# JitongZ/shockwave-replication

Hardware: AMD Instinct MI355X
Metric: Shockwave plan solves/sec at 900 jobs x 30 rounds (higher is better)
Workload: dtype f64 objective / fp32 ranking keys

## Files before the change

### shockwave-replication_amd/csrc/sw_block.h

```cpp
#pragma once
#include <hip/hip_runtime.h>
#include <stdint.h>

#define SW_BLOCK 512
#define SW_WAVES (SW_BLOCK / 64)

template <int NW>
struct sw_xchg_t {
    int64_t i[2][NW][2];
    double d[2][NW][2];
    uint64_t u[2][NW];
    uint64_t u2[2][NW][2];
    int32_t s[2][NW];
};
using sw_xchg = sw_xchg_t<SW_WAVES>;

__device__ __forceinline__ int lane_id() { return threadIdx.x & 63; }
__device__ __forceinline__ int wave_id() { return threadIdx.x >> 6; }

__device__ __forceinline__ int32_t sw_u32(int32_t x) { return __builtin_amdgcn_readfirstlane(x); }
__device__ __forceinline__ uint64_t sw_u64(uint64_t x) {
    const uint32_t lo = (uint32_t)__builtin_amdgcn_readfirstlane((int)(uint32_t)x);
    const uint32_t hi = (uint32_t)__builtin_amdgcn_readfirstlane((int)(uint32_t)(x >> 32));
    return ((uint64_t)hi << 32) | lo;
}
__device__ __forceinline__ int64_t sw_i64(int64_t x) { return (int64_t)sw_u64((uint64_t)x); }
__device__ __forceinline__ double sw_f64u(double x) {
    return __builtin_bit_cast(double, sw_u64(__builtin_bit_cast(uint64_t, x)));
}

__device__ __forceinline__ void wave_sync() {
    __builtin_amdgcn_fence(__ATOMIC_SEQ_CST, "wavefront");
    __builtin_amdgcn_wave_barrier();
}

__device__ __forceinline__ int32_t dpp_incscan_i32(int32_t x) {
    x += __builtin_amdgcn_update_dpp(0, x, 0x111, 0xF, 0xF, false);
    x += __builtin_amdgcn_update_dpp(0, x, 0x112, 0xF, 0xF, false);
    x += __builtin_amdgcn_update_dpp(0, x, 0x114, 0xF, 0xF, false);
    x += __builtin_amdgcn_update_dpp(0, x, 0x118, 0xF, 0xF, false);
    x += __builtin_amdgcn_update_dpp(0, x, 0x142, 0xA, 0xF, false);
    x += __builtin_amdgcn_update_dpp(0, x, 0x143, 0xC, 0xF, false);
    return x;
}
__device__ __forceinline__ int32_t dpp_incmax_i32(int32_t x) {
    const int32_t lo = INT32_MIN;
    int32_t y;
    y = __builtin_amdgcn_update_dpp(lo, x, 0x111, 0xF, 0xF, false); x = y > x ? y : x;
    y = __builtin_amdgcn_update_dpp(lo, x, 0x112, 0xF, 0xF, false); x = y > x ? y : x;
    y = __builtin_amdgcn_update_dpp(lo, x, 0x114, 0xF, 0xF, false); x = y > x ? y : x;
    y = __builtin_amdgcn_update_dpp(lo, x, 0x118, 0xF, 0xF, false); x = y > x ? y : x;
    y = __builtin_amdgcn_update_dpp(lo, x, 0x142, 0xA, 0xF, false); x = y > x ? y : x;
    y = __builtin_amdgcn_update_dpp(lo, x, 0x143, 0xC, 0xF, false); x = y > x ? y : x;
    return x;
}
__device__ __forceinline__ int32_t wave_sum_i32(int32_t v) {
    return __builtin_amdgcn_readlane(dpp_incscan_i32(v), 63);
}
__device__ __forceinline__ int32_t wave_max_i32(int32_t v) {
    return __builtin_amdgcn_readlane(dpp_incmax_i32(v), 63);
}
__device__ __forceinline__ int32_t wave_min_i32(int32_t v) {
    return -wave_max_i32(-v);
}
__device__ __forceinline__ int32_t wave_incscan_i32(int32_t v) { return dpp_incscan_i32(v); }
__device__ __forceinline__ int32_t wave_sufscan_i32(int32_t v) {
    const int32_t inc = dpp_incscan_i32(v);
    return __builtin_amdgcn_readlane(inc, 63) - inc + v;
}

#define SW_DPP64(x, idv, ctrl, rm)                                                              \
    ((((uint64_t)(uint32_t)__builtin_amdgcn_update_dpp((int)(uint32_t)((idv) >> 32),            \
                                                       (int)(uint32_t)((x) >> 32), ctrl, rm,    \
                                                       0xF, false)) << 32) |                    \
     (uint64_t)(uint32_t)__builtin_amdgcn_update_dpp((int)(uint32_t)(idv), (int)(uint32_t)(x),  \
                                                     ctrl, rm, 0xF, false))
#define SW_DPP64_STEPS(STEP) STEP(0x111, 0xF) STEP(0x112, 0xF) STEP(0x114, 0xF) STEP(0x118, 0xF) \
    STEP(0x142, 0xA) STEP(0x143, 0xC)

__device__ __forceinline__ uint64_t sw_readlane63_u64(uint64_t x) {
    const uint32_t lo = (uint32_t)__builtin_amdgcn_readlane((int)(uint32_t)x, 63);
    const uint32_t hi = (uint32_t)__builtin_amdgcn_readlane((int)(uint32_t)(x >> 32), 63);
    return ((uint64_t)hi << 32) | lo;
}
__device__ __forceinline__ uint64_t wave_max_u64(uint64_t x) {
#define SW_MAXU_(c, rm)                               \
    {                                                 \
        const uint64_t y_ = SW_DPP64(x, 0ull, c, rm); \
        x = y_ > x ? y_ : x;                          \
    }
    SW_DPP64_STEPS(SW_MAXU_)
#undef SW_MAXU_
    return sw_readlane63_u64(x);
}
__device__ __forceinline__ uint64_t wave_min_u64(uint64_t x) {
#define SW_MINU_(c, rm)                                \
    {                                                  \
        const uint64_t y_ = SW_DPP64(x, ~0ull, c, rm); \
        x = y_ < x ? y_ : x;                           \
    }
    SW_DPP64_STEPS(SW_MINU_)
#undef SW_MINU_
    return sw_readlane63_u64(x);
}
__device__ __forceinline__ double wave_max_f64(double v) {
    uint64_t x = __builtin_bit_cast(uint64_t, v);
#define SW_MAXD_(c, rm)                                                       \
    {                                                                         \
        const uint64_t y_ = SW_DPP64(x, 0xFFF0000000000000ull, c, rm);        \
        x = __builtin_bit_cast(double, y_) > __builtin_bit_cast(double, x) ? y_ : x; \
    }
    SW_DPP64_STEPS(SW_MAXD_)
#undef SW_MAXD_
    return __builtin_bit_cast(double, sw_readlane63_u64(x));
}

__device__ __forceinline__ double wave_min_f64(double v) {
    uint64_t x = __builtin_bit_cast(uint64_t, v);
#define SW_MIND_(c, rm)                                                       \
    {                                                                         \
        const uint64_t y_ = SW_DPP64(x, 0x7FF0000000000000ull, c, rm);        \
        x = __builtin_bit_cast(double, y_) < __builtin_bit_cast(double, x) ? y_ : x; \
    }
    SW_DPP64_STEPS(SW_MIND_)
#undef SW_MIND_
    return __builtin_bit_cast(double, sw_readlane63_u64(x));
}

template <typename T>
__device__ __forceinline__ T wave_sum(T v) {
#pragma unroll
    for (int o = 32; o >= 1; o >>= 1) v += __shfl_xor(v, o, 64);
    return v;
}

template <typename T>
__device__ __forceinline__ T wave_max(T v) {
#pragma unroll
    for (int o = 32; o >= 1; o >>= 1) {
        T x = __shfl_xor(v, o, 64);
        v = x > v ? x : v;
    }
    return v;
}

template <typename T>
__device__ __forceinline__ T wave_min(T v) {
#pragma unroll
    for (int o = 32; o >= 1; o >>= 1) {
        T x = __shfl_xor(v, o, 64);
        v = x < v ? x : v;
    }
    return v;
}

template <typename T>
__device__ __forceinline__ T wave_incscan(T v) {
    const int lane = lane_id();
#pragma unroll
    for (int o = 1; o < 64; o <<= 1) {
        T y = __shfl_up(v, o, 64);
        if (lane >= o) v += y;
    }
    return v;
}

template <typename T>
__device__ __forceinline__ T wave_sufscan(T v) {
    const int lane = lane_id();
#pragma unroll
    for (int o = 1; o < 64; o <<= 1) {
        T y = __shfl_down(v, o, 64);
        if (lane + o < 64) v += y;
    }
    return v;
}

__device__ __forceinline__ int32_t wave_sort_asc_i32(int32_t v) {
    const int lane = lane_id();
#pragma unroll
    for (int k = 2; k <= 64; k <<= 1) {
#pragma unroll
        for (int j = k >> 1; j > 0; j >>= 1) {
            const int32_t o = __shfl_xor(v, j, 64);
            const bool up = (lane & k) == 0;
// ... 274 lines not shown
```

### shockwave-replication_amd/csrc/sw_kernels.hip

```cpp
#include <hip/hip_runtime.h>
#include <stdint.h>

#include "../../include/shockwave_amd.h"
#include "sw_arith.h"
#include "sw_rowsearch.h"
#include "sw_block.h"
#include "sw_device.h"
#include "sw_pack.h"
#include "sw_bnb.h"
#include "sw_repair.h"
#include "sw_reround_dev.h"
#include "sw_p2x_inst.h"

namespace {

#ifdef SW_STAMPS
#define SW_STAMP(slot)                                                            \
    do {                                                                          \
        __syncthreads();                                                          \
        if (threadIdx.x == 0 && B.stamps) {                                       \
            uint64_t now_ = __builtin_amdgcn_s_memtime();                         \
            B.stamps[(size_t)inst_ * SW_STAMP_SLOTS + (slot)] += now_ - stamp_prev_;      \
            stamp_prev_ = now_;                                                   \
        }                                                                         \
// ... 1706 lines not shown
        v.bound = bound;
        v.passes = c.passes;
        B.lvl[inst_] = v;
    }
}

__device__ __forceinline__ void emit_plan_bytes(uint8_t* plan, const uint64_t* ym, int N, int T) {
    const int32_t nbytes = N * T;
    const int32_t mis = (int32_t)(reinterpret_cast<uintptr_t>(plan) & 15u);
    const int32_t head = min(nbytes, (16 - mis) & 15);
    const int32_t nch = (nbytes - head) >> 4;
    auto byte_at = [&](int32_t b) {
        const int32_t j = b / T;
        return (uint8_t)((ym[j] >> (b - j * T)) & 1ull);
    };
    for (int32_t b = threadIdx.x; b < head; b += SW_BLOCK) plan[b] = byte_at(b);
    for (int32_t b = head + nch * 16 + threadIdx.x; b < nbytes; b += SW_BLOCK) plan[b] = byte_at(b);
    uint4* dst = reinterpret_cast<uint4*>(plan + head);
    for (int32_t ci = threadIdx.x; ci < nch; ci += SW_BLOCK) {
        const int32_t b0 = head + ci * 16;
        int32_t j = b0 / T, t = b0 - j * T;
        uint64_t m = ym[j];
        uint32_t wv[4] = {0u, 0u, 0u, 0u};
#pragma unroll
        for (int k = 0; k < 16; ++k) {
            wv[k >> 2] |= (uint32_t)((m >> t) & 1ull) << ((k & 3) * 8);
            if (++t == T) {
                t = 0;
                ++j;
                if (k < 15 && j < N) m = ym[j];
            }
        }
        dst[ci] = make_uint4(wv[0], wv[1], wv[2], wv[3]);
    }
}

__device__ __forceinline__ void emit_out(sw_out_dev* out, double U, double M, double k, double P2,
                                         double bound, int64_t passes, int32_t status) {
    sw_out_dev o;
    o.objective = U - k * M;
    o.utility = U;
    o.makespan = M;
    o.p2_objective = P2;
    o.bound = bound;
    o.iters = (int32_t)passes;
    o.status = status | (sw_p1_uncertified(o.objective, bound) ? SW_STATUS_P1_UNCERTIFIED : 0);
    *out = o;
}

static_assert(SW_LDS_JOBS <= (1 << 11), "the job index fits the position word");
#define SW_LWA_MARKED (-1)

template <bool WS>
__device__ __forceinline__ const uint64_t* pack_instance(const sw_batch_dev& B, unsigned char* smem, int inst_) {
    const sw_inst_dev* I = &B.inst[inst_];
    Ctx<32, true, true> c;
    c.init(B, I);
    const sw_lvl_dev lv = B.lvl[inst_];
    c.passes = lv.passes;
    const int64_t jo = I->job_off;
    constexpr sw_pack_carve O = sw_pack_offsets();
    c.blk.X = (sw_xchg*)(smem + O.X);
    c.set_pack_lds(smem + O.PL);
    c.misc = (int64_t*)(smem + O.misc);
    c.rep = (sw_repair_t*)(smem + O.rep);
    c.nbest = smem + O.nbest;
    c.placed = smem + O.placed;
    c.placed2 = smem + O.placed2;
    c.ycur = (uint64_t*)(smem + O.ycur);
    c.y2 = (uint64_t*)(smem + O.y2);
    c.sbuf = (uint64_t*)(smem + O.sbuf);
    sw_out_dev* out = &B.out[inst_];
    if constexpr (!WS) {
        int64_t act_l = 0;
        c.for_jobs([&](int j, int s) {
            (void)s;
            c.nbest[j] = B.nb[jo + j];
            act_l += c.nbest[j] > 0;
        });
        if (c.blk.sum(act_l) > SW_BLOCK) {
            if (threadIdx.x == 0) out->status = SW_STATUS_SLOW_MARK;
            return nullptr;
        }
        c.pack(4, c.nbest, c.ycur, c.placed);
    } else {
        const int A_ = sw_u32(B.lwa[inst_]);
        if (A_ == SW_LWA_MARKED) return nullptr;
        c.for_jobs([&](int j, int s) {
            (void)s;
            c.nbest[j] = B.nb[jo + j];
            c.ycur[j] = 0;
        });
        const bool mine = (int)threadIdx.x < A_;
        const uint32_t word = mine ? B.lws[jo + threadIdx.x] : 0u;
        const uint64_t mk1 = mine ? B.lwm[jo + threadIdx.x] : 0ull;
        c.pack_back(4, c.nbest, c.ycur, c.placed, mine, (int)(word >> 16), word & 0xFFFFu, mk1);
    }
    int64_t def_l = 0;
    c.for_jobs([&](int j, int s) {
        (void)s;
        def_l += (int64_t)c.w_in[j] * (c.nbest[j] - c.placed[j]);
    });
    int64_t dfc = c.blk.sum(def_l);
    c.passes++;
    int32_t status = 0;
    if (dfc != 0 && c.repair_pack(c.nbest, c.ycur, c.placed, c.y2, c.placed2)) {
        c.for_jobs([&](int j, int s) {
            (void)s;
            c.ycur[j] = c.y2[j];
        });
        c.passes++;
        dfc = 0;
        status |= SW_STATUS_P2_REPAIRED;
    }
    if (dfc != 0) {
        if (threadIdx.x == 0) out->status = SW_STATUS_SLOW_MARK;
        return nullptr;
    }
    int64_t any_l = 0;
    double p2 = 0.0;
    c.for_jobs([&](int j, int s) {
        (void)s;
        const uint64_t m = c.ycur[j];
        const int cnt = __popcll(m);
        any_l += (cnt > 0);
        p2 = p2 + (cnt > 0 ? sw_p2_term(m, cnt, c.p_in[j]) : 0.0);
        B.planned[jo + j] = cnt;
    });
    const double P2 = c.blk.detsum(p2);
    const int64_t any_n = c.blk.sum(any_l);
    if (any_n == 0) status |= SW_STATUS_NO_PLANNED;
    if (threadIdx.x == 0) emit_out(out, lv.U, lv.M, c.k, P2, lv.bound, c.passes, status);
    return c.ycur;
}

__device__ __forceinline__ void pack_tail(const sw_batch_dev& B, const uint64_t* ym, unsigned char* smem,
                                          int inst) {
    const sw_inst_dev* I = &B.inst[inst];
    sw_out_dev* out = &B.out[inst];
    const int N = I->N, T = I->T, G = I->G;
    const int64_t jo = I->job_off;
    const int q = (N + SW_BLOCK - 1) / SW_BLOCK;
    const int j0 = sw_tid_opaque() * q, j1 = min(j0 + q, N);
    __syncthreads();
    int act = 0;
#pragma unroll
    for (int k = 0; k < 2; ++k) act += (j0 + k < j1 && ym[j0 + k] != 0ull) ? 1 : 0;
    const bool run = B.fuse_p2x && !(out->status & SW_STATUS_P2_FALLBACK);
    sw_p2x_lds* L = reinterpret_cast<sw_p2x_lds*>(smem);
    const size_t Lsz = SW_P2X_VAR_OFF;
    unsigned char* var = smem + Lsz;
    static_assert(offsetof(sw_p2x_lds, X) + sizeof(sw_xchg) <= sw_pack_offsets().ycur,
                  "the pack's masks lie past the exchange words of sw_p2x_lds");
    sw_blk blk;
    blk.X = &L->X;
    blk.par = 0;
    int A = 0;
    const int a0 = blk.exscan(act, A);
    A = __builtin_amdgcn_readfirstlane(A);
    const uint64_t* yemit = ym;
    if (run && A > 0 && A <= SW_P2X_AMAX) {
        const size_t vb = (sw_p2x_var_bytes(A, T) + 15) & ~(size_t)15;
        const bool onchip = Lsz + vb + (size_t)SW_P2X_ARR_BYTES * A <= (size_t)B.lds_bytes &&
                            var + vb >= reinterpret_cast<const unsigned char*>(ym + N);
        unsigned char* base = onchip ? var + vb : B.p2ws + (size_t)SW_P2X_ARR_BYTES * jo;
        const size_t n = onchip ? (size_t)A : (size_t)N;
        const sw_p2x_arrays X = sw_p2x_view(base, n);
        for (int k = 0, a = a0; k < 2; ++k) {
            if (j0 + k >= j1) break;
            const uint64_t m = ym[j0 + k];
            if (m == 0ull) continue;
            const int j = j0 + k;
            X.cw[a] = B.w[jo + j];
            X.cj[a] = j;
            X.cc[a] = B.p[jo + j] / (double)__popcll(m);
            X.cm[a] = m;
            ++a;
        }
        __syncthreads();
#ifdef SW_STAMPS
        uint64_t* sp = B.stamps ? B.stamps + (size_t)inst * SW_STAMP_SLOTS + 32 : nullptr;
#else
        uint64_t* sp = nullptr;
#endif
        const int nc = sw_p2x_block<SW_WAVES>(blk, L, var, X, A, T, G, sp);
        __syncthreads();
        int act2 = 0;
        for (int j = j0r(N); j < j1r(N); ++j) act2 += B.planned[jo + j] > 0;
        int A2;
        int a = blk.exscan(act2, A2);
        uint64_t mf[2];
        double acc = 0.0;
#pragma unroll
        for (int k = 0; k < 2; ++k) {
            const int j = j0r(N) + k;
            mf[k] = 0ull;
            if (j >= j1r(N)) continue;
            if (B.planned[jo + j] <= 0) {
                acc = acc + 0.0;
                continue;
            }
            mf[k] = X.cm[a++];
            acc = acc + sw_p2_term(mf[k], __popcll(mf[k]), B.p[jo + j]);
        }
        if (nc > 0) {
            const double P2 = blk.detsum(acc);
            if (threadIdx.x == 0) {
                out->p2_objective = P2;
                out->status |= SW_STATUS_P2_EXCHANGED;
            }
        }
        __syncthreads();
        uint64_t* yf = reinterpret_cast<uint64_t*>(smem);
#pragma unroll
        for (int k = 0; k < 2; ++k)
            if (j0r(N) + k < j1r(N)) yf[j0r(N) + k] = mf[k];
        yemit = yf;
        __syncthreads();
    }
    if (B.want_masks)
        for (int j = j0r(N); j < j1r(N); ++j) B.masks[jo + j] = yemit[j];
    emit_plan_bytes(B.plan + I->plan_off, yemit, N, T);
}

template <int KT, bool ONE>
struct RREnv {
    Ctx<KT, ONE>& c;
    sw_blk& blk;
    int N, T, G;
    double k;
    uint8_t *S, *Sb;
    uint32_t* items;
    double *iv, *dpA, *dpB;
    uint64_t* bits;
    double rv[SW_JPT], r0[SW_JPT], r1[SW_JPT];
    double *gv, *g0, *g1;
    __device__ RREnv(Ctx<KT, ONE>& cc) : c(cc), blk(cc.blk) {}
    template <class F>
    __device__ __forceinline__ void for_jobs(F&& f) { c.for_jobs(f); }
    __device__ __forceinline__ sw_jobc jc(int j) const { return c.jc(j, 0); }
    __device__ __forceinline__ double f(const sw_jobc& q, int n) const {
        return sw_f(&q, n, c.nb, c.beta, c.ell, c.slope);
    }
    __device__ __forceinline__ bool tj(int j) const { return c.jc(j, 0).w <= G; }
    __device__ __forceinline__ uint64_t& y(int j) { return c.ybest[j]; }
    __device__ __forceinline__ int cnt(int j) const { return c.nfin[j]; }
    __device__ __forceinline__ void add_cnt(int j, int d) { c.nfin[j] = (uint8_t)(c.nfin[j] + d); }
    __device__ __forceinline__ double& V(int j, int s) {
        if constexpr (ONE) { (void)j; return rv[s]; } else { (void)s; return gv[j]; }
    }
    __device__ __forceinline__ double& H0(int j, int s) {
        if constexpr (ONE) { (void)j; return r0[s]; } else { (void)s; return g0[j]; }
    }
    __device__ __forceinline__ double& H1(int j, int s) {
        if constexpr (ONE) { (void)j; return r1[s]; } else { (void)s; return g1[j]; }
    }
};

template <int KT, bool ONE>
__device__ __forceinline__ int reround(Ctx<KT, ONE>& c, double* rr_dpA, double* rr_dpB, uint64_t* rr_bits) {
    RREnv<KT, ONE> e(c);
    e.N = c.N;
    e.T = c.T;
    e.G = c.G;
    e.k = c.k;
    e.S = c.placed;
    e.Sb = c.placed2;
    if constexpr (ONE) {
// ... 386 lines not shown
```

### shockwave-replication_amd/csrc/sw_p2x_dev.h

```cpp
#pragma once
#include <hip/hip_runtime.h>
#include <stdint.h>

#include "../../include/shockwave_amd.h"
#include "sw_arith.h"
#include "sw_block.h"
#include "sw_device.h"
#include "sw_p2x.h"

struct sw_p2x_arrays {
    int32_t* cw;
    int32_t* cj;
    double* cc;
    uint64_t* cm;
};
static_assert(SW_P2X_ARR_BYTES == 2 * sizeof(int32_t) + sizeof(double) + sizeof(uint64_t),
              "SW_P2X_ARR_BYTES (sw_p2x.h) must cover the sw_p2x_arrays layout");

struct sw_p2x_pre {
    const int32_t* hdr;
    const int32_t* ord;
    const double* pc;
    const uint64_t* B;
    const double* Wb;
    const int8_t* Wk;
};
enum { SW_P2X_HDR_K = 0, SW_P2X_HDR_WC = 1, SW_P2X_HDR_M = 9, SW_P2X_HDR_OFF = 17,
       SW_P2X_HDR_NW = 26, SW_P2X_HDR_BOFF = 34, SW_P2X_HDR_A = 42, SW_P2X_HDR_INTS = 48 };

struct sw_p2x_lds {
    sw_xchg X;
    int32_t wc[SW_P2X_KMAX], M[SW_P2X_KMAX], off[SW_P2X_KMAX + 1], nw[SW_P2X_KMAX],
        boff[SW_P2X_KMAX];
    int32_t K, len, nrec, pad;
    uint64_t touched;
    uint32_t wmap[8];
    int32_t room[SW_TMAX];
    int32_t pr[SW_TMAX + 1];
    int32_t cyc[SW_TMAX + 2];
    double delta;
    double bd[SW_TMAX + 1];
    int32_t bp[SW_TMAX + 1];
    double pv[SW_WAVES][64];
    int8_t pt[SW_WAVES][64];
    int32_t bfdone;
    int32_t fq[SW_P2X_KMAX];
    double dw[SW_P2X_KMAX][SW_TMAX + 1];
};

__host__ __device__ inline size_t sw_p2x_var_bytes(int maxA, int T) {
    const size_t a = (size_t)(maxA < SW_P2X_AMAX ? maxA : SW_P2X_AMAX);
    const size_t words = (size_t)T * ((a + 63) / 64 + SW_P2X_KMAX);
    size_t np = 1;
    while (np < a) np <<= 1;
    const size_t work = words * 8 + (size_t)T * T * 8 + (((size_t)T * T + 15) & ~(size_t)15) +
                        (size_t)SW_P2X_MAX_MOVES * 4;
    return a * 8 + ((a * 4 + 15) & ~(size_t)15) + (work > 16 * np ? work : 16 * np);
}

static __device__ __forceinline__ int p2x_class(const sw_p2x_lds* L, int32_t w) {
    int k = 0;
    while (k < L->K - 1 && L->wc[k] != w) ++k;
    return k;
}

static __device__ __forceinline__ void p2x_find_cycle(sw_p2x_lds* L, const double* W, int T, int F,
                                                      double* dw, bool warm, uint64_t (&acc)[11]) {
    const int tid = threadIdx.x, lane = lane_id(), wv = wave_id();
    (void)acc;
#ifdef SW_STAMPS
    uint64_t bt_ = __builtin_amdgcn_s_memtime();
#define BF_STAMP(k)                                                   \
    do {                                                              \
        const uint64_t now_ = __builtin_amdgcn_s_memtime();           \
        acc[k] += now_ - bt_;                                         \
        bt_ = now_;                                                   \
    } while (0)
#else
#define BF_STAMP(k) \
    do {            \
    } while (0)
#endif
    const bool act = lane < T;
    if (tid <= T) {
        L->bd[tid] = warm ? dw[tid] : 0.0;
        L->bp[tid] = -1;
    }
    if (tid == 0) L->bfdone = 0;
    const bool roomok = wv == 0 && act && L->room[lane] >= F;
    const bool anyroom = __ballot(roomok) != 0;
    const int nq = (T + SW_WAVES - 1) / SW_WAVES;
    int ndbl = 0;
    while ((1 << ndbl) < T + 1) ++ndbl;
    __syncthreads();
    for (int it = 0; it <= T; ++it) {
#ifdef SW_STAMPS
        acc[7] += 1;
#endif
        BF_STAMP(10);
        {
            const int ul = act ? lane : 0;
            const int t0 = wv * nq, t1 = min(T, t0 + nq);
            double cb = SW_P2X_NONE;
            int ct = 0;
            for (int t = t0; t < t1; ++t) {
                const double w = W[t * T + ul];
                const double v = L->bd[t] + w;
                const bool take = w < SW_P2X_NONE && v < cb;
                cb = take ? v : cb;
                ct = take ? t : ct;
            }
            L->pv[wv][lane] = cb;
            L->pt[wv][lane] = (int8_t)ct;
        }
        __syncthreads();
        BF_STAMP(9);
        if (wv == 0) {
            __builtin_amdgcn_s_setprio(3);
            double d = act ? L->bd[lane] : 0.0;
// ... 223 lines not shown
        sp_t_ = now_;                                                \
    } while (0)
#else
#define P2X_STAMP(k) \
    do {             \
    } while (0)
#endif

template <int NT, int EMAX>
static __device__ __forceinline__ void p2x_sort_regs(uint64_t (&hi)[EMAX], uint64_t (&lo)[EMAX], int E,
                                                     int np, uint64_t* xs) {
    const int tid = threadIdx.x;
    for (int kk = 2; kk <= np; kk <<= 1) {
        for (int jj = kk >> 1; jj > 0; jj >>= 1) {
            if (jj < E) {
#pragma unroll
                for (int e = 0; e < EMAX; ++e) {
                    const int f = e ^ jj;
                    if (e < E && f > e) {
                        const int i = tid * E + e;
                        const bool up = (i & kk) == 0;
                        uint64_t ah = hi[e], al = lo[e], bh = 0, bl = 0;
#pragma unroll
                        for (int g = 0; g < EMAX; ++g)
                            if (g == f) { bh = hi[g]; bl = lo[g]; }
                        const bool gt = ah > bh || (ah == bh && al > bl);
                        if (up == gt) {
                            hi[e] = bh; lo[e] = bl;
#pragma unroll
                            for (int g = 0; g < EMAX; ++g)
                                if (g == f) { hi[g] = ah; lo[g] = al; }
                        }
                    }
                }
            } else {
                uint64_t ph[EMAX], pl[EMAX];
                const int dj = jj / E;
                if (dj < 64) {
#pragma unroll
                    for (int e = 0; e < EMAX; ++e) {
                        ph[e] = __shfl_xor(hi[e], dj, 64);
                        pl[e] = __shfl_xor(lo[e], dj, 64);
                    }
                } else {
                    if (tid * E < np)
                        for (int e = 0; e < E; ++e) {
                            xs[tid * E + e] = hi[e];
                            xs[np + tid * E + e] = lo[e];
                        }
                    __syncthreads();
                    const int pt = tid ^ dj;
                    if (tid * E < np)
                        for (int e = 0; e < E; ++e) {
                            ph[e] = xs[pt * E + e];
                            pl[e] = xs[np + pt * E + e];
                        }
                    __syncthreads();
                }
                const bool lower = (tid & dj) == 0;
#pragma unroll
                for (int e = 0; e < EMAX; ++e) {
                    if (e >= E) continue;
                    const int i = tid * E + e;
                    const bool up = (i & kk) == 0;
                    const bool gt = hi[e] > ph[e] || (hi[e] == ph[e] && lo[e] > pl[e]);
                    if ((lower == up) ? gt : !gt) {
                        hi[e] = ph[e];
                        lo[e] = pl[e];
                    }
                }
            }
        }
    }
}

struct sw_p2x_state {
    int K;
    double* pc;
    int32_t* ord;
    uint64_t* B;
    double* W;
    int8_t* Wk;
    double delta;
};

static __device__ __forceinline__ void p2x_load_size(sw_p2x_lds* L, int K, int F) {
    const int tid = threadIdx.x;
    if (tid < SW_P2X_KMAX) {
        const int wk = tid < K ? L->wc[tid] : 0;
        L->fq[tid] = (wk > 0 && wk <= F && F % wk == 0 && F / wk <= SW_P2X_QMAX) ? F / wk : 0;
    }
}

template <int NW, int EMAX = 1, bool SETUP_ONLY = false>
__device__ __forceinline__ int sw_p2x_block(sw_blk_t<NW>& blk, sw_p2x_lds* L, unsigned char* var,
                                            const sw_p2x_arrays& X, int A, int T, int G,
                                            uint64_t* sp = nullptr, const sw_p2x_pre* pre = nullptr,
                                            sw_p2x_state* st = nullptr) {
    constexpr int NT = NW * 64;
    const int tid = threadIdx.x;
    (void)sp;
    uint64_t sp_a_[11] = {0, 0, 0, 0, 0, 0, 0, 0, 0, 0, 0};
#ifdef SW_STAMPS
    uint64_t sp_t_ = __builtin_amdgcn_s_memtime();
#endif
    if (A <= 0 || T < 2 || A > SW_P2X_AMAX) return 0;
    if (pre && pre->hdr[SW_P2X_HDR_K] < 0) return 0;
    if (pre) {
        if (tid < SW_P2X_KMAX) {
            L->wc[tid] = pre->hdr[SW_P2X_HDR_WC + tid];
            L->M[tid] = pre->hdr[SW_P2X_HDR_M + tid];
            L->nw[tid] = pre->hdr[SW_P2X_HDR_NW + tid];
            L->boff[tid] = pre->hdr[SW_P2X_HDR_BOFF + tid];
        }
        if (tid <= SW_P2X_KMAX) L->off[tid] = pre->hdr[SW_P2X_HDR_OFF + tid];
        if (tid == 0) L->K = pre->hdr[SW_P2X_HDR_K];
        __syncthreads();
    }
    if (!pre) {
    if (tid < 8) L->wmap[tid] = 0u;
    __syncthreads();
    for (int a = tid; a < A; a += NT) atomicOr(&L->wmap[X.cw[a] >> 5], 1u << (X.cw[a] & 31));
    __syncthreads();
    if (tid == 0) {
        int K = 0;
        for (int i = 0; i < 8; ++i) K += __builtin_popcount(L->wmap[i]);
        if (K > SW_P2X_KMAX) {
            L->K = -1;
        } else {
            K = 0;
            for (int i = 0; i < 8; ++i)
                for (uint32_t b = L->wmap[i]; b; b &= b - 1) L->wc[K++] = 32 * i + __builtin_ctz(b);
            L->K = K;
            for (int k = 0; k < K; ++k) L->M[k] = 0;
        }
    }
    __syncthreads();
    if (L->K < 0) return 0;
    for (int a = tid; a < A; a += NT) atomicAdd(&L->M[p2x_class(L, X.cw[a])], 1);
    __syncthreads();
    if (tid == 0) {
        const int K = L->K;
        int o = 0, b = 0;
        for (int k = 0; k < K; ++k) {
            L->off[k] = o;
            L->nw[k] = (L->M[k] + 63) / 64;
            L->boff[k] = b;
            o += L->M[k];
            b += L->nw[k] * T;
        }
        L->off[K] = o;
    }
    }
    const int K = L->K;
    P2X_STAMP(0);
    double* pc = reinterpret_cast<double*>(var);
    int32_t* ord = reinterpret_cast<int32_t*>(var + (size_t)A * 8);
    unsigned char* vb = var + (size_t)A * 8 + (((size_t)A * 4 + 15) & ~(size_t)15);
    __syncthreads();
    const int nwords = L->boff[K - 1] + L->nw[K - 1] * T;
    uint64_t* B = reinterpret_cast<uint64_t*>(vb);
    double* W = reinterpret_cast<double*>(vb + (size_t)nwords * 8);
    int8_t* Wk = reinterpret_cast<int8_t*>(W + T * T);
    int32_t* rec = reinterpret_cast<int32_t*>(reinterpret_cast<unsigned char*>(Wk) + ((T * T + 15) & ~15));
    if (pre) {
        for (int p = tid; p < A; p += NT) {
            ord[p] = pre->ord[p];
            pc[p] = pre->pc[p];
        }
        for (int i = tid; i < nwords; i += NT) B[i] = pre->B[i];
        __syncthreads();
    } else if (A <= NT) {
        int np = 1;
        while (np < A) np <<= 1;
        uint64_t hi = ~0ull, lo = ~0ull;
        if (tid < A) {
            const uint64_t ck = sw_p2x_ckey(X.cc[tid]);
            hi = ((uint64_t)p2x_class(L, X.cw[tid]) << 61) | (~ck & ((1ull << 61) - 1));
            lo = ((uint64_t)(uint32_t)X.cj[tid] << 32) | (uint32_t)tid;
        }
        uint64_t* xs = reinterpret_cast<uint64_t*>(vb);
        for (int kk = 2; kk <= np; kk <<= 1) {
            for (int jj = kk >> 1; jj > 0; jj >>= 1) {
                uint64_t ph = ~0ull, pl = ~0ull;
                if (jj >= 64) {
                    if (tid < np) {
                        xs[tid] = hi;
                        xs[np + tid] = lo;
                    }
                    __syncthreads();
                    if (tid < np) {
                        ph = xs[tid ^ jj];
                        pl = xs[np + (tid ^ jj)];
                    }
                    __syncthreads();
                } else {
                    ph = __shfl_xor(hi, jj, 64);
                    pl = __shfl_xor(lo, jj, 64);
                }
                const bool up = (tid & kk) == 0, lower = (tid & jj) == 0;
                const bool gt = hi > ph || (hi == ph && lo > pl);
                if ((lower == up) ? gt : !gt) {
                    hi = ph;
                    lo = pl;
                }
            }
        }
        if (tid < A) {
            const int a = (int)(uint32_t)lo;
            ord[tid] = a;
            pc[tid] = X.cc[a];
        }
        __syncthreads();
    } else if (EMAX > 1 && A <= EMAX * NT) {
        int np = 1;
        while (np < A) np <<= 1;
        const int E = np / NT;
        uint64_t hi[EMAX], lo[EMAX];
#pragma unroll
        for (int e = 0; e < EMAX; ++e) {
            const int i = tid * E + e;
            hi[e] = ~0ull;
            lo[e] = ~0ull;
            if (e < E && i < A) {
                const uint64_t ck = sw_p2x_ckey(X.cc[i]);
                hi[e] = ((uint64_t)p2x_class(L, X.cw[i]) << 61) | (~ck & ((1ull << 61) - 1));
                lo[e] = ((uint64_t)(uint32_t)X.cj[i] << 32) | (uint32_t)i;
            }
        }
        p2x_sort_regs<NT, EMAX>(hi, lo, E, np, reinterpret_cast<uint64_t*>(vb));
#pragma unroll
        for (int e = 0; e < EMAX; ++e) {
            const int p = tid * E + e;
            if (e < E && p < A) {
                const int a = (int)(uint32_t)lo[e];
                ord[p] = a;
                pc[p] = X.cc[a];
            }
        }
        __syncthreads();
    } else {
        int np = 1;
        while (np < A) np <<= 1;
        uint64_t* k1 = reinterpret_cast<uint64_t*>(vb);
        uint32_t* k2 = reinterpret_cast<uint32_t*>(k1 + np);
        uint32_t* ka = k2 + np;
        for (int i = tid; i < np; i += NT) {
            if (i < A) {
                const uint64_t ck = sw_p2x_ckey(X.cc[i]);
                k1[i] = ((uint64_t)p2x_class(L, X.cw[i]) << 61) | (~ck & ((1ull << 61) - 1));
                k2[i] = (uint32_t)X.cj[i];
                ka[i] = (uint32_t)i;
            } else {
                k1[i] = ~0ull;
                k2[i] = 0xFFFFFFFFu;
                ka[i] = 0u;
            }
        }
        __syncthreads();
        const int chunk = np / NW;
        const int lane = lane_id(), wv = wave_id();
        for (int k = 2; k <= np; k <<= 1) {
            for (int j = k >> 1; j > 0; j >>= 1) {
                const bool local = j < chunk;
                const int x0 = local ? lane : tid, xs = local ? 64 : NT;
                const int nx = local ? (chunk >> 1) : (np >> 1), base = local ? wv * chunk : 0;
                for (int x = x0; x < nx; x += xs) {
                    const int i = base + 2 * x - (x & (j - 1)), l = i + j;
                    const uint64_t a1 = k1[i], b1 = k1[l];
                    const uint32_t a2 = k2[i], b2 = k2[l];
                    const bool gt = a1 > b1 || (a1 == b1 && a2 > b2);
                    if (((i & k) == 0) == gt) {
                        k1[i] = b1; k1[l] = a1;
                        k2[i] = b2; k2[l] = a2;
                        const uint32_t t = ka[i]; ka[i] = ka[l]; ka[l] = t;
                    }
                }
                const int nj = j > 1 ? (j >> 1) : k;
                const bool next_local = (j > 1 || (k << 1) <= np) && nj < chunk;
                if (local && next_local) wave_sync();
                else __syncthreads();
            }
        }
        for (int p = tid; p < A; p += NT) {
            const int a = (int)ka[p];
            ord[p] = a;
            pc[p] = X.cc[a];
        }
        __syncthreads();
    }
    P2X_STAMP(1);
    {
        const int lane = lane_id(), wv = wave_id();
        int nslot = 0;
        for (int k = 0; k < K; ++k) nslot += L->nw[k];
        if (pre) nslot = 0;
        for (int sl = wv; sl < nslot; sl += NW) {
            int k = 0, w = sl;
            while (w >= L->nw[k]) w -= L->nw[k++];
            const int r = 64 * w + lane;
            const uint64_t m = r < L->M[k] ? X.cm[ord[L->off[k] + r]] : 0ull;
            uint64_t* Bk = B + L->boff[k] + (size_t)w * T;
            for (int t = 0; t < T; ++t) {
                const uint64_t word = __ballot((m >> t) & 1ull);
                if (lane == 0) Bk[t] = word;
            }
        }
        __syncthreads();
        if (tid < T) {
            int32_t used = 0;
            for (int k = 0; k < K; ++k) {
                const uint64_t* Bk = B + L->boff[k] + tid;
                int32_t c = 0;
                for (int w = 0; w < L->nw[k]; ++w) c += __popcll(Bk[w * T]);
                used += c * L->wc[k];
            }
            L->room[tid] = G - used;
        }
    }
    {
        const int q = (A + SW_DET_LANES - 1) / SW_DET_LANES;
        static_assert(NT == SW_DET_LANES, "one thread per deterministic-sum lane");
        double acc = 0.0;
        for (int p = tid * q; p < A && p < (tid + 1) * q; ++p) {
            int64_t S = 0;
            for (uint64_t x = X.cm[ord[p]]; x; x &= x - 1) S += __builtin_ctzll(x);
            acc = acc + pc[p] * (double)S;
        }
        const double P0 = blk.detsum(acc);
        if (tid == 0) L->delta = sw_p2x_delta(P0, T, A);
    }
    __syncthreads();
    const double delta = L->delta;
    P2X_STAMP(2);
    if constexpr (SETUP_ONLY) {
        st->K = K;
        st->pc = pc;
        st->ord = ord;
        st->B = B;
        st->W = W;
        st->Wk = Wk;
        st->delta = delta;
        return 1;
    }
    int ncancel = 0;
    int cert[SW_P2X_KMAX];
#pragma unroll
    for (int k = 0; k < SW_P2X_KMAX; ++k) cert[k] = -1;
    uint32_t havem = 0;
    for (bool changed = true; changed && ncancel < SW_P2X_MAX_CANCEL;) {
        changed = false;
        for (int ki = 0; ki < K && ncancel < SW_P2X_MAX_CANCEL; ++ki) {
            const int F = L->wc[ki];
            int certk = -1;
#pragma unroll
            for (int k = 0; k < SW_P2X_KMAX; ++k) certk = k == ki ? cert[k] : certk;
            if (certk == ncancel) continue;
            p2x_load_size(L, K, F);
            __syncthreads();
            bool all = true;
            while (ncancel < SW_P2X_MAX_CANCEL) {
                if (pre && all && ncancel == 0) {
                    const double* Wb = pre->Wb + (size_t)ki * T * T;
                    const int8_t* Wkb = pre->Wk + (size_t)ki * T * T;
                    for (int e = tid; e < T * T; e += NT) {
                        const double b = Wb[e];
                        W[e] = b < SW_P2X_NONE ? b + delta : SW_P2X_NONE;
                        Wk[e] = Wkb[e];
                    }
                } else {
                    p2x_build_w<NT>(L, B, pc, W, Wk, T, delta, all);
                }
                __syncthreads();
                P2X_STAMP(3);
                sp_a_[8] += 1;
                p2x_find_cycle(L, W, T, F, L->dw[ki], ((havem >> ki) & 1u) != 0, sp_a_);
                havem |= 1u << ki;
                P2X_STAMP(4);
                const int len = L->len;
                if (len == 0) {
#pragma unroll
                    for (int k = 0; k < SW_P2X_KMAX; ++k) cert[k] = k == ki ? ncancel : cert[k];
                    break;
                }
                if (wave_id() == 0) {
                    const int lane = lane_id();
                    int moves = 0;
                    uint64_t tm = 0;
                    for (int b0 = 0; b0 < len; b0 += 64) {
                        const int i = b0 + lane;
                        const int u = i < len ? L->cyc[i] : T, t = i < len ? L->cyc[(i + 1) % len] : T;
                        const bool real = u < T && t < T;
                        const int q = real ? F / L->wc[Wk[t * T + u]] : 0;
                        moves += wave_sum_i32(q);
                    }
                    int n0 = 0;
                    for (int b0 = 0; b0 < len; b0 += 64) {
                        const int i = b0 + lane;
                        const int u = i < len ? L->cyc[i] : T, t = i < len ? L->cyc[(i + 1) % len] : T;
                        const bool real = u < T && t < T;
                        const int k = real ? Wk[t * T + u] : 0;
                        const int q = real ? F / L->wc[k] : 0;
                        const int incl = wave_incscan_i32(q);
                        if (real) tm |= (1ull << t) | (1ull << u);
                        if (real && moves <= SW_P2X_MAX_MOVES) {
                            const uint64_t* Bt = B + L->boff[k] + t;
                            const uint64_t* Bu = B + L->boff[k] + u;
                            int r = sw_p2x_start(Bt, Bu, L->nw[k], T, q, u < t);
                            int n = n0 + incl - q;
                            for (int g = 0; g < q; ++g) {
                                rec[n++] = (k << 29) | (t << 23) | (u << 17) | r;
                                if (g + 1 < q) r = sw_p2x_next(Bt, Bu, L->nw[k], T, r + 1);
                            }
                        }
                        n0 += __shfl(incl, 63, 64);
                    }
                    for (int o = 32; o >= 1; o >>= 1) {
                        const uint64_t v = (uint64_t)__shfl_xor((long long)tm, o, 64);
                        tm |= v;
                    }
                    if (lane == 0) {
                        L->nrec = moves <= SW_P2X_MAX_MOVES ? n0 : -1;
                        L->touched = tm;
                    }
                }
                __syncthreads();
                P2X_STAMP(5);
                const int nrec = L->nrec;
                if (nrec < 0) break;
                for (int i = tid; i < nrec; i += NT) {
                    const int32_t v = rec[i];
                    const int k = (v >> 29) & 7, t = (v >> 23) & 63, u = (v >> 17) & 63, r = v & 0x1FFFF;
                    uint64_t* Bk = B + L->boff[k];
                    const uint64_t bit = 1ull << (r & 63);
                    atomicAnd((unsigned long long*)&Bk[(r >> 6) * T + t], ~bit);
                    atomicOr((unsigned long long*)&Bk[(r >> 6) * T + u], bit);
                    atomicXor((unsigned long long*)&X.cm[ord[L->off[k] + r]], (1ull << t) | (1ull << u));
                    atomicAdd(&L->room[t], L->wc[k]);
                    atomicAdd(&L->room[u], -L->wc[k]);
                }
                __syncthreads();
                P2X_STAMP(6);
                ++ncancel;
                changed = true;
                all = false;
            }
        }
    }
#ifdef SW_STAMPS
    if (threadIdx.x == 0 && sp)
        for (int k = 0; k < 11; ++k) sp[k] += sp_a_[k];
#endif
    return ncancel;
}
```

Measured before the change: 2.973 million.

## Reuse packing candidate order to rank p2x classes and build classes with wave ballots

```diff
diff --git a/shockwave-replication_amd/csrc/sw_block.h b/shockwave-replication_amd/csrc/sw_block.h
--- a/shockwave-replication_amd/csrc/sw_block.h
+++ b/shockwave-replication_amd/csrc/sw_block.h
@@ -101,6 +101,12 @@
     }
     SW_DPP64_STEPS(SW_MINU_)
 #undef SW_MINU_
+    return sw_readlane63_u64(x);
+}
+__device__ __forceinline__ uint64_t wave_or_u64(uint64_t x) {
+#define SW_ORU_(c, rm) x |= SW_DPP64(x, 0ull, c, rm);
+    SW_DPP64_STEPS(SW_ORU_)
+#undef SW_ORU_
     return sw_readlane63_u64(x);
 }
 __device__ __forceinline__ double wave_max_f64(double v) {
diff --git a/shockwave-replication_amd/csrc/sw_kernels.hip b/shockwave-replication_amd/csrc/sw_kernels.hip
--- a/shockwave-replication_amd/csrc/sw_kernels.hip
+++ b/shockwave-replication_amd/csrc/sw_kernels.hip
@@ -1812,7 +1812,17 @@
             if (threadIdx.x == 0) out->status = SW_STATUS_SLOW_MARK;
             return nullptr;
         }
-        c.pack(4, c.nbest, c.ycur, c.placed);
+        __syncthreads();
+        uint64_t khi[SW_JPT], klo[SW_JPT];
+        int A_, jp1 = 0;
+        bool mine = false;
+        uint32_t st1 = 0u;
+        c.pack_front(4, c.nbest, c.ycur, khi, klo, A_, mine, jp1, st1);
+        if (mine) B.lws[jo + threadIdx.x] = st1 | ((uint32_t)jp1 << 16);
+        if (threadIdx.x == 0) B.lwa[inst_] = A_;
+        uint64_t mk1 = 0ull;
+        c.pack_loop(4, A_, st1, mk1);
+        c.pack_back(4, c.nbest, c.ycur, c.placed, mine, jp1, st1, mk1);
     } else {
         const int A_ = sw_u32(B.lwa[inst_]);
         if (A_ == SW_LWA_MARKED) return nullptr;
@@ -1913,7 +1923,12 @@
 #else
         uint64_t* sp = nullptr;
 #endif
-        const int nc = sw_p2x_block<SW_WAVES>(blk, L, var, X, A, T, G, sp);
+        sw_p2x_cand cand;
+        cand.pos = B.lws + jo;
+        cand.n = sw_u32(B.lwa[inst]);
+        cand.njobs = N;
+        const int nc = sw_p2x_block<SW_WAVES>(blk, L, var, X, A, T, G, sp, nullptr, nullptr,
+                                              &cand);
         __syncthreads();
         int act2 = 0;
         for (int j = j0r(N); j < j1r(N); ++j) act2 += B.planned[jo + j] > 0;
diff --git a/shockwave-replication_amd/csrc/sw_p2x_dev.h b/shockwave-replication_amd/csrc/sw_p2x_dev.h
--- a/shockwave-replication_amd/csrc/sw_p2x_dev.h
+++ b/shockwave-replication_amd/csrc/sw_p2x_dev.h
@@ -7,6 +7,7 @@
 #include "sw_block.h"
 #include "sw_device.h"
 #include "sw_p2x.h"
+#include "sw_p2x_rank.h"
 
 struct sw_p2x_arrays {
     int32_t* cw;
@@ -28,13 +29,17 @@
 enum { SW_P2X_HDR_K = 0, SW_P2X_HDR_WC = 1, SW_P2X_HDR_M = 9, SW_P2X_HDR_OFF = 17,
        SW_P2X_HDR_NW = 26, SW_P2X_HDR_BOFF = 34, SW_P2X_HDR_A = 42, SW_P2X_HDR_INTS = 48 };
 
+struct sw_p2x_cand {
+    const uint32_t* pos;
+    int32_t n, njobs;
+};
+
 struct sw_p2x_lds {
     sw_xchg X;
     int32_t wc[SW_P2X_KMAX], M[SW_P2X_KMAX], off[SW_P2X_KMAX + 1], nw[SW_P2X_KMAX],
         boff[SW_P2X_KMAX];
     int32_t K, len, nrec, pad;
     uint64_t touched;
-    uint32_t wmap[8];
     int32_t room[SW_TMAX];
     int32_t pr[SW_TMAX + 1];
     int32_t cyc[SW_TMAX + 2];
@@ -424,6 +429,7 @@
     double* W;
     int8_t* Wk;
     double delta;
+    int ranked;
 };
 
 static __device__ __forceinline__ void p2x_load_size(sw_p2x_lds* L, int K, int F) {
@@ -434,11 +440,143 @@
     }
 }
 
+template <int NW>
+static __device__ __forceinline__ void p2x_classes(sw_p2x_lds* L, const int32_t* cw, int A, int T) {
+    constexpr int NT = NW * 64, KM = SW_P2X_KMAX, NONE = 0x7FFFFFFF;
+    static_assert(NW * KM <= 64 && (2 * NW * KM + NW) * 4 <= (int)sizeof(L->pv),
+                  "one lane of wave 0 per list entry; the lists fit L->pv");
+    const int lane = lane_id(), wv = wave_id();
+    int32_t* wl = reinterpret_cast<int32_t*>(&L->pv[0][0]);
+    int32_t* cl = wl + NW * KM;
+    int32_t* ov = cl + NW * KM;
+    int lw = NONE, lc = 0, nl = 0;
+    bool over = false;
+    for (int a0 = wv * 64; a0 < A && !over; a0 += NT) {
+        const int a = a0 + lane;
+        const int w = a < A ? cw[a] : 0;
+        uint64_t rem = __ballot(a < A);
+        while (rem) {
+            const int w0 = __builtin_amdgcn_readlane(w, (int)__builtin_ctzll(rem));
+            const uint64_t same = __ballot(w == w0) & rem;
+            rem &= ~same;
+            if (__ballot(lw == w0) != 0) {
+                lc += lw == w0 ? __popcll(same) : 0;
+            } else if (nl < KM) {
+                if (lane == nl) {
+                    lw = w0;
+                    lc = __popcll(same);
+                }
+                ++nl;
+            } else {
+                over = true;
+                rem = 0;
+            }
+        }
+    }
+    if (lane < KM) {
+        wl[wv * KM + lane] = lw;
+        cl[wv * KM + lane] = lc;
+    }
+    if (lane == 0) ov[wv] = over ? 1 : 0;
+    __syncthreads();
+    if (wv == 0) {
+        int w = lane < NW * KM ? wl[lane] : NONE;
+        const int c = lane < NW * KM ? cl[lane] : 0;
+        int K = __ballot(lane < NW && ov[lane] != 0) != 0 ? KM + 1 : 0;
+        int myw = 0, myM = 0;
+        while (K <= KM) {
+            const int wmin = wave_min_i32(w);
+            if (wmin == NONE) break;
+            const bool s = w == wmin;
+            const int m = wave_sum_i32(s ? c : 0);
+            if (lane == K) {
+                myw = wmin;
+                myM = m;
+            }
+            w = s ? NONE : w;
+            ++K;
+        }
+        if (K > KM) {
+            if (lane == 0) L->K = -1;
+        } else {
+            const int nwk = (myM + 63) / 64;
+            const int incM = wave_incscan_i32(myM), incB = wave_incscan_i32(nwk * T);
+            if (lane < K) {
+                L->wc[lane] = myw;
+                L->M[lane] = myM;
+                L->nw[lane] = nwk;
+                L->boff[lane] = incB - nwk * T;
+            }
+            if (lane <= K) L->off[lane] = incM - myM;
+            if (lane == 0) L->K = K;
+        }
+    }
+    __syncthreads();
+}
+
+template <int NW>
+static __device__ __forceinline__ bool p2x_rank_from(sw_blk_t<NW>& blk, sw_p2x_lds* L, unsigned char* xs,
+                                                     size_t room, const sw_p2x_arrays& X, int A, int K,
+                                                     const sw_p2x_cand& cand, int32_t* ord, double* pc) {
+    constexpr int KM = SW_P2X_KMAX;
+    const int tid = threadIdx.x, lane = lane_id(), wv = wave_id();
+    const int nj = cand.njobs;
+    if (cand.n != A || nj <= 0 || sw_p2x_rank_bytes(A, nj) > room) return false;
+    uint64_t* skey = reinterpret_cast<uint64_t*>(xs);
+    int32_t* sjob = reinterpret_cast<int32_t*>(xs + (((size_t)A * 8 + 15) & ~(size_t)15));
+    uint16_t* j2a = reinterpret_cast<uint16_t*>(reinterpret_cast<unsigned char*>(sjob) +
+                                                (((size_t)A * 4 + 15) & ~(size_t)15));
+    int32_t* cnt = reinterpret_cast<int32_t*>(&L->pv[0][0]);
+    const bool mine = tid < A;
+    const int job = mine ? (int)(cand.pos[tid] >> 16) : 0;
+    if (mine) {
+        const int j = X.cj[tid];
+        if ((unsigned)j < (unsigned)nj) j2a[j] = (uint16_t)tid;
+    }
+    __syncthreads();
+    bool ok = true;
+    int a = 0, k = 0;
+    if (mine) {
+        ok = job < nj;
+        a = ok ? (int)j2a[job] : 0;
+        ok = ok && a < A;
+        a = ok ? a : 0;
+        ok = ok && X.cj[a] == job;
+        k = p2x_class(L, X.cw[a]);
+    }
+    int r = 0;
+    for (int kk = 0; kk < K; ++kk) {
+        const uint64_t same = __ballot(mine && k == kk);
+        r = k == kk ? sw_p2x_rank_lane(same, lane) : r;
+        if (lane == 0) cnt[wv * KM + kk] = __popcll(same);
+    }
+    __syncthreads();
+    for (int w = 0; w < wv; ++w) r += cnt[w * KM + k];
+    const int dst = mine ? sw_p2x_rank_dst(L->off, k, r) : 0;
+    ok = ok && dst >= 0;
+    const double c = X.cc[a];
+    if (mine && ok) {
+        skey[dst] = sw_p2x_ckey(c);
+        sjob[dst] = job;
+    }
+    __syncthreads();
+    if (mine && ok) ok = sw_p2x_rank_ok(skey, sjob, L->off, k, dst) != 0;
+    const bool all = blk.min32(ok ? 1 : 0) != 0;
+    if (all) {
+        if (mine) {
+            ord[dst] = a;
+            pc[dst] = c;
+        }
+        __syncthreads();
+    }
+    return all;
+}
+
 template <int NW, int EMAX = 1, bool SETUP_ONLY = false>
 __device__ __forceinline__ int sw_p2x_block(sw_blk_t<NW>& blk, sw_p2x_lds* L, unsigned char* var,
                                             const sw_p2x_arrays& X, int A, int T, int G,
                                             uint64_t* sp = nullptr, const sw_p2x_pre* pre = nullptr,
-                                            sw_p2x_state* st = nullptr) {
+                                            sw_p2x_state* st = nullptr, const sw_p2x_cand* cand = nullptr) {
     constexpr int NT = NW * 64;
     const int tid = threadIdx.x;
     (void)sp;
@@ -460,51 +598,20 @@
         __syncthreads();
     }
     if (!pre) {
-    if (tid < 8) L->wmap[tid] = 0u;
-    __syncthreads();
-    for (int a = tid; a < A; a += NT) atomicOr(&L->wmap[X.cw[a] >> 5], 1u << (X.cw[a] & 31));
-    __syncthreads();
-    if (tid == 0) {
-        int K = 0;
-        for (int i = 0; i < 8; ++i) K += __builtin_popcount(L->wmap[i]);
-        if (K > SW_P2X_KMAX) {
-            L->K = -1;
-        } else {
-            K = 0;
-            for (int i = 0; i < 8; ++i)
-                for (uint32_t b = L->wmap[i]; b; b &= b - 1) L->wc[K++] = 32 * i + __builtin_ctz(b);
-            L->K = K;
-            for (int k = 0; k < K; ++k) L->M[k] = 0;
-        }
-    }
-    __syncthreads();
+    p2x_classes<NW>(L, X.cw, A, T);
     if (L->K < 0) return 0;
-    for (int a = tid; a < A; a += NT) atomicAdd(&L->M[p2x_class(L, X.cw[a])], 1);
-    __syncthreads();
-    if (tid == 0) {
-        const int K = L->K;
-        int o = 0, b = 0;
-        for (int k = 0; k < K; ++k) {
-            L->off[k] = o;
-            L->nw[k] = (L->M[k] + 63) / 64;
-            L->boff[k] = b;
-            o += L->M[k];
-            b += L->nw[k] * T;
-        }
-        L->off[K] = o;
-    }
     }
     const int K = L->K;
     P2X_STAMP(0);
     double* pc = reinterpret_cast<double*>(var);
     int32_t* ord = reinterpret_cast<int32_t*>(var + (size_t)A * 8);
     unsigned char* vb = var + (size_t)A * 8 + (((size_t)A * 4 + 15) & ~(size_t)15);
-    __syncthreads();
     const int nwords = L->boff[K - 1] + L->nw[K - 1] * T;
     uint64_t* B = reinterpret_cast<uint64_t*>(vb);
     double* W = reinterpret_cast<double*>(vb + (size_t)nwords * 8);
     int8_t* Wk = reinterpret_cast<int8_t*>(W + T * T);
     int32_t* rec = reinterpret_cast<int32_t*>(reinterpret_cast<unsigned char*>(Wk) + ((T * T + 15) & ~15));
+    bool ranked = false;
     if (pre) {
         for (int p = tid; p < A; p += NT) {
             ord[p] = pre->ord[p];
@@ -512,6 +619,10 @@
         }
         for (int i = tid; i < nwords; i += NT) B[i] = pre->B[i];
         __syncthreads();
+    } else if (A <= NT && cand &&
+               p2x_rank_from<NW>(blk, L, vb, sw_p2x_var_bytes(A, T) - (size_t)(vb - var), X, A, K, *cand, ord,
+                                 pc)) {
+        ranked = true;
     } else if (A <= NT) {
         int np = 1;
         while (np < A) np <<= 1;
@@ -665,9 +776,7 @@
         static_assert(NT == SW_DET_LANES, "one thread per deterministic-sum lane");
         double acc = 0.0;
         for (int p = tid * q; p < A && p < (tid + 1) * q; ++p) {
-            int64_t S = 0;
-            for (uint64_t x = X.cm[ord[p]]; x; x &= x - 1) S += __builtin_ctzll(x);
-            acc = acc + pc[p] * (double)S;
+            acc = acc + pc[p] * (double)sw_mask_tsum(X.cm[ord[p]]);
         }
         const double P0 = blk.detsum(acc);
         if (tid == 0) L->delta = sw_p2x_delta(P0, T, A);
@@ -683,6 +792,7 @@
         st->W = W;
         st->Wk = Wk;
         st->delta = delta;
+        st->ranked = ranked ? 1 : 0;
         return 1;
     }
     int ncancel = 0;
@@ -733,7 +843,7 @@
                         const int i = b0 + lane;
                         const int u = i < len ? L->cyc[i] : T, t = i < len ? L->cyc[(i + 1) % len] : T;
                         const bool real = u < T && t < T;
-                        const int q = real ? F / L->wc[Wk[t * T + u]] : 0;
+                        const int q = real ? L->fq[Wk[t * T + u]] : 0;
                         moves += wave_sum_i32(q);
                     }
                     int n0 = 0;
@@ -742,7 +852,7 @@
                         const int u = i < len ? L->cyc[i] : T, t = i < len ? L->cyc[(i + 1) % len] : T;
                         const bool real = u < T && t < T;
                         const int k = real ? Wk[t * T + u] : 0;
-                        const int q = real ? F / L->wc[k] : 0;
+                        const int q = real ? L->fq[k] : 0;
                         const int incl = wave_incscan_i32(q);
                         if (real) tm |= (1ull << t) | (1ull << u);
                         if (real && moves <= SW_P2X_MAX_MOVES) {
@@ -757,10 +867,7 @@
                         }
                         n0 += __shfl(incl, 63, 64);
                     }
-                    for (int o = 32; o >= 1; o >>= 1) {
-                        const uint64_t v = (uint64_t)__shfl_xor((long long)tm, o, 64);
-                        tm |= v;
-                    }
+                    tm = wave_or_u64(tm);
                     if (lane == 0) {
                         L->nrec = moves <= SW_P2X_MAX_MOVES ? n0 : -1;
                         L->touched = tm;
diff --git a/shockwave-replication_amd/csrc/sw_p2x_rank.h b/shockwave-replication_amd/csrc/sw_p2x_rank.h
--- /dev/null
+++ b/shockwave-replication_amd/csrc/sw_p2x_rank.h
@@ -0,0 +1,62 @@
+#ifndef SW_P2X_RANK_H
+#define SW_P2X_RANK_H
+
+#include <stddef.h>
+#include <stdint.h>
+
+#include "sw_arith.h"
+
+SW_HD int sw_p2x_rank_before(uint64_t ka, int32_t ja, uint64_t kb, int32_t jb) {
+    return ka > kb || (ka == kb && ja < jb);
+}
+
+SW_HD int32_t sw_p2x_rank_lane(uint64_t same, int32_t lane) {
+    return (int32_t)__builtin_popcountll(same & ((1ull << (lane & 63)) - 1ull));
+}
+
+SW_HD int32_t sw_p2x_rank_dst(const int32_t* off, int32_t k, int32_t r) {
+    const int32_t d = off[k] + r;
+    return d < off[k + 1] ? d : -1;
+}
+
+SW_HD int sw_p2x_rank_ok(const uint64_t* skey, const int32_t* sjob, const int32_t* off, int32_t k,
+                         int32_t dst) {
+    return dst == off[k] || sw_p2x_rank_before(skey[dst - 1], sjob[dst - 1], skey[dst], sjob[dst]);
+}
+
+SW_HD size_t sw_p2x_rank_bytes(int32_t A, int32_t njobs) {
+    return (((size_t)A * 8 + 15) & ~(size_t)15) + (((size_t)A * 4 + 15) & ~(size_t)15) +
+           (((size_t)njobs * 2 + 15) & ~(size_t)15);
+}
+
+SW_HD int sw_p2x_rank_place(int32_t n, int32_t A, int32_t K, const int32_t* off, const int32_t* cls,
+                            const uint64_t* ckey, const int32_t* job, int32_t* dst, uint64_t* skey,
+                            int32_t* sjob) {
+    int32_t cnt[8];
+    int ok = 1;
+    if (n != A || K < 1 || K > 8) return 0;
+    for (int32_t k = 0; k < K; ++k) cnt[k] = 0;
+    for (int32_t q0 = 0; q0 < n; q0 += 64) {
+        const int32_t m = n - q0 < 64 ? n - q0 : 64;
+        for (int32_t k = 0; k < K; ++k) {
+            uint64_t same = 0;
+            for (int32_t l = 0; l < m; ++l) same |= (uint64_t)(cls[q0 + l] == k) << l;
+            for (int32_t l = 0; l < m; ++l)
+                if (cls[q0 + l] == k) dst[q0 + l] = sw_p2x_rank_dst(off, k, cnt[k] + sw_p2x_rank_lane(same, l));
+            cnt[k] += (int32_t)__builtin_popcountll(same);
+        }
+    }
+    for (int32_t q = 0; q < n; ++q) {
+        if (dst[q] < 0) {
+            ok = 0;
+            continue;
+        }
+        skey[dst[q]] = ckey[q];
+        sjob[dst[q]] = job[q];
+    }
+    if (!ok) return 0;
+    for (int32_t q = 0; q < n; ++q) ok &= sw_p2x_rank_ok(skey, sjob, off, cls[q], dst[q]);
+    return ok;
+}
+
+#endif
```

After: 3.087 million, median of 6. +3.8%, better.
